# jcmgray/cotengra

Hardware: NVIDIA H100
Metric: sycamore_n53_m20_sliced_contract_tflops (higher is better)
Workload: dtype c128 (f64 arithmetic)

## Files before the change

### cotengra_b200/csrc/rowstream.cuh

```cuda
#pragma once

template <typename T, int NMAX, int KMAX, bool BREG, bool STRIP = false>
__global__ void __launch_bounds__(256, BREG ? 2 : 3)
rowstream_kernel(const int64_t* __restrict__ D, const T* __restrict__ A, const T* __restrict__ B, T* __restrict__ C) {
  STREAM_TABLES(T, KMAX, NMAX, KMAX);
  const int tid = threadIdx.x;
  const int K = (int)D[W_KTA], N = (int)D[W_NTA];
  const StreamFlags f = stream_flags<T>(D);
  const int n_m = s.load(D, B, K, N);
  [[maybe_unused]] T breg[BREG ? KMAX : 1][BREG ? NMAX : 1];
  if constexpr (BREG) {
#pragma unroll
    for (int kk = 0; kk < KMAX; ++kk)
#pragma unroll
      for (int c = 0; c < NMAX; ++c) breg[kk][c] = s.B[kk * NMAX + c];
  }
  long long akoff[KMAX];
#pragma unroll
  for (int kk = 0; kk < KMAX; ++kk) akoff[kk] = s.akoff[kk];

  [[maybe_unused]] StripCtx sctx;
  if constexpr (STRIP) sctx = strip_begin(D);
  const unsigned long long M = (unsigned long long)D[W_MTA] * (unsigned long long)D[W_TILES_M];
  const unsigned long long stride = (unsigned long long)gridDim.x * blockDim.x;
  constexpr int R = sizeof(T) >= 16 ? 1 : ((sizeof(T) == 8 && KMAX <= 4) ? 4 : 2);
  for (unsigned long long m0 = (unsigned long long)blockIdx.x * blockDim.x + tid; m0 < M; m0 += stride * R) {
    long long oa[R], oc[R];
    bool live[R];
#pragma unroll
    for (int i = 0; i < R; ++i) {
      const unsigned long long m = m0 + (unsigned long long)i * stride;
      live[i] = m < M;
      s.row(n_m, f.pow2, live[i] ? (unsigned)m : 0u, oa[i], oc[i]);
    }
    T a[R][KMAX];
#pragma unroll
    for (int i = 0; i < R; ++i)
#pragma unroll
      for (int kk = 0; kk < KMAX; ++kk)
        if (kk < K) a[i][kk] = A[oa[i] + akoff[kk]];
    [[maybe_unused]] int sb0 = 0;
    if constexpr (!BREG && sizeof(T) >= 16) asm volatile("" : "+r"(sb0));
    constexpr int CH = (NMAX > 4 && sizeof(T) >= 16) ? 4 : NMAX;
#pragma unroll
    for (int i = 0; i < R; ++i) {
      if (!live[i]) continue;
      T* pc = C + oc[i];
#pragma unroll
      for (int c0 = 0; c0 < NMAX; c0 += CH) {
        if (c0 >= N) break;
        T acc[CH];
#pragma unroll
        for (int c = 0; c < CH; ++c) acc[c] = zero_of<T>();
#pragma unroll
        for (int kk = 0; kk < KMAX; ++kk) {
          if (kk < K) {
#pragma unroll
            for (int c = 0; c < CH; ++c) {
              if constexpr (BREG) {
                mac(acc[c], a[i][kk], breg[kk][c0 + c]);
              } else {
                if (c0 + c < N) mac(acc[c], a[i][kk], s.B[sb0 + kk * NMAX + c0 + c]);
              }
            }
          }
        }
        if constexpr (STRIP) strip_row(sctx, acc, c0, N);
        store_row<true>(pc, s.cnoff, acc, c0, N, f);
      }
    }
  }
  if constexpr (STRIP) strip_end(sctx);
}

constexpr int RSK_KMAX = 64, RSK_NMAX = 8;

template <typename T, bool STRIP = false>
__global__ void __launch_bounds__(256, 3)
rowstream_longk_kernel(const int64_t* __restrict__ D, const T* __restrict__ A, const T* __restrict__ B,
                       T* __restrict__ C) {
  STREAM_TABLES(T, RSK_KMAX, RSK_NMAX, RSK_KMAX);
  const int tid = threadIdx.x;
  const int K = (int)D[W_KTA], N = (int)D[W_NTA];
  const StreamFlags f = stream_flags<T>(D);
  const int n_m = s.load(D, B, K, N);
  long long inoff[8];
#pragma unroll
  for (int kk = 0; kk < 8; ++kk) inoff[kk] = s.akoff[kk];
  const int nchunks = (K + 7) >> 3;
  [[maybe_unused]] StripCtx sctx;
  if constexpr (STRIP) sctx = strip_begin(D);
  const unsigned long long M = (unsigned long long)D[W_MTA] * (unsigned long long)D[W_TILES_M];
  const unsigned long long stride = (unsigned long long)gridDim.x * blockDim.x;
  constexpr int R = 2;
  for (unsigned long long m0 = (unsigned long long)blockIdx.x * blockDim.x + tid; m0 < M; m0 += stride * R) {
    long long oa[R], oc[R];
    bool live[R];
#pragma unroll
    for (int i = 0; i < R; ++i) {
      const unsigned long long m = m0 + (unsigned long long)i * stride;
      live[i] = m < M;
      s.template row<false>(n_m, f.pow2, live[i] ? (unsigned)m : 0u, oa[i], oc[i]);
    }
    T acc[R][RSK_NMAX];
#pragma unroll
    for (int i = 0; i < R; ++i)
#pragma unroll
      for (int c = 0; c < RSK_NMAX; ++c) acc[i][c] = zero_of<T>();
    for (int kc = 0; kc < nchunks; ++kc) {
      const long long cb = s.akoff[kc * 8];
      T a[R][8];
#pragma unroll
      for (int i = 0; i < R; ++i)
#pragma unroll
        for (int kk = 0; kk < 8; ++kk) a[i][kk] = (kc * 8 + kk < K) ? A[oa[i] + cb + inoff[kk]] : zero_of<T>();
#pragma unroll
      for (int kk = 0; kk < 8; ++kk)
#pragma unroll
        for (int c = 0; c < RSK_NMAX; ++c) {
          const T b = s.B[(kc * 8 + kk) * RSK_NMAX + c];
#pragma unroll
          for (int i = 0; i < R; ++i) mac(acc[i][c], a[i][kk], b);
        }
    }
#pragma unroll
    for (int i = 0; i < R; ++i) {
      if (!live[i]) continue;
      if constexpr (STRIP) strip_row(sctx, acc[i], 0, N);
      store_row<false>(C + oc[i], s.cnoff, acc[i], 0, N, f);
    }
  }
  if constexpr (STRIP) strip_end(sctx);
}
```

Measured before the change: 25.28.

## Transpose complex output rows through shared memory for coalesced C stores

For complex types with an 8-wide N and no register-held B, each warp writes its per-row accumulators into a swizzled shared-memory tile and then stores them back so that consecutive lanes write different columns of the same rows. This replaces strided per-thread row stores with more coalesced global writes. It adds shared memory per block, warp syncs and shuffles, and keeps whole warps alive in the loop so the shuffles stay valid, which may lower occupancy.

Result: faster. 25.78, median of 6 (+2.0%).

```diff
diff --git a/cotengra_b200/csrc/rowstream.cuh b/cotengra_b200/csrc/rowstream.cuh
--- a/cotengra_b200/csrc/rowstream.cuh
+++ b/cotengra_b200/csrc/rowstream.cuh
@@ -24,7 +24,15 @@
   const unsigned long long M = (unsigned long long)D[W_MTA] * (unsigned long long)D[W_TILES_M];
   const unsigned long long stride = (unsigned long long)gridDim.x * blockDim.x;
   constexpr int R = sizeof(T) >= 16 ? 1 : ((sizeof(T) == 8 && KMAX <= 4) ? 4 : 2);
-  for (unsigned long long m0 = (unsigned long long)blockIdx.x * blockDim.x + tid; m0 < M; m0 += stride * R) {
+  constexpr bool XPOSE = sizeof(T) >= 16 && NMAX == 8 && !BREG;
+  [[maybe_unused]] T* xrows = nullptr;
+  const unsigned lane = tid & 31;
+  if constexpr (XPOSE) {
+    __shared__ T s_rows[256 * 8];
+    xrows = s_rows + (tid >> 5) * 32 * 8;
+  }
+  const unsigned long long lane0 = XPOSE ? lane : 0;
+  for (unsigned long long m0 = (unsigned long long)blockIdx.x * blockDim.x + tid; m0 - lane0 < M; m0 += stride * R) {
     long long oa[R], oc[R];
     bool live[R];
 #pragma unroll
@@ -44,7 +52,7 @@
     constexpr int CH = (NMAX > 4 && sizeof(T) >= 16) ? 4 : NMAX;
 #pragma unroll
     for (int i = 0; i < R; ++i) {
-      if (!live[i]) continue;
+      if (!XPOSE && !live[i]) continue;
       T* pc = C + oc[i];
 #pragma unroll
       for (int c0 = 0; c0 < NMAX; c0 += CH) {
@@ -65,9 +73,33 @@
             }
           }
         }
-        if constexpr (STRIP) strip_row(sctx, acc, c0, N);
-        store_row<true>(pc, s.cnoff, acc, c0, N, f);
+        if constexpr (STRIP) {
+          if (!XPOSE || live[i]) strip_row(sctx, acc, c0, N);
+        }
+        if constexpr (XPOSE) {
+#pragma unroll
+          for (int c = 0; c < CH; ++c) xrows[lane * 8 + ((c0 + c) ^ (lane & 7))] = acc[c];
+        } else {
+          store_row<true>(pc, s.cnoff, acc, c0, N, f);
+        }
       }
+    }
+    if constexpr (XPOSE) {
+      __syncwarp();
+      const unsigned long long mw = m0 - lane;
+      const int j = lane & 7;
+      const long long cj = s.cnoff[j];
+#pragma unroll
+      for (int q = 0; q < 8; ++q) {
+        const int r = q * 4 + (lane >> 3);
+        const long long ocr = __shfl_sync(0xffffffffu, oc[0], r);
+        if (mw + r < M && j < N) {
+          const T v = xrows[r * 8 + (j ^ (r & 7))];
+          T* p = C + ocr + cj;
+          *p = f.accumulate ? add_of(*p, v) : v;
+        }
+      }
+      __syncwarp();
     }
   }
   if constexpr (STRIP) strip_end(sctx);
```
